# hahnyuan/PTQ4ViT

Hardware: AMD Instinct MI355X
Metric: calibration throughput (wrapped modules calibrated per second), ViT-B/224 W8A8, 32 calibration images (higher is better)
Workload: dtype int8

## Files before the change

include/ptq4vit_hip_debug.h:

```cpp
#ifndef PTQ4VIT_HIP_DEBUG_H
#define PTQ4VIT_HIP_DEBUG_H

#include <stdint.h>

#ifdef __cplusplus
extern "C" {
#endif

int p4v_debug_set_variant(int variant, int force_generic);
int p4v_debug_set_tuning(int key, int value);
int p4v_debug_topk_rows(const float* d_mass, int segs, int n, int k, int32_t* d_idx, void* stream);
int p4v_debug_pack_dual(const float* d_x, long rows, long cols, long cols_padded, int sos, int lo, int hi, int qmax,
                        const float* d_scale, float const_scale, int8_t* d_q1, int8_t* d_q2, void* stream);
int p4v_debug_pack_cands(const float* d_x, long rows, long cols, long rows_padded, long cols_padded, int layout, int lo, int hi,
                         const float* d_scales, int n_cands, const int* d_crange, const unsigned char* d_done, int live_max,
                         int general, int8_t* d_q, void* stream);
int p4v_debug_gather_im2col(int batch, int in_channels, int height, int width, int kernel_h, int kernel_w, int stride_h, int stride_w,
                            int pad_h, int pad_w, int dil_h, int dil_w, const float* d_x, const int32_t* d_idx, int k, float* d_dst,
                            void* stream);
int p4v_debug_prep_epi6(const float* d_o, const float* d_wt, const float* d_bias, long o_ss, long o_ts, int sr, int tr,
                        int bias_on_t, int wt_mode, int transposed, float* d_e, void* stream);

#ifdef __cplusplus
}
#endif
#endif
```

ptq4vit_amd/_lib.py:

```python
import ctypes as C
import os

_HERE = os.path.dirname(os.path.abspath(__file__))
LIB_PATH = os.environ.get("P4V_LIB") or os.path.join(_HERE, "csrc", "libptq4vit_hip.so")

METRICS = {
    "L1_norm": 0,
    "L2_norm": 1,
    "linear_weighted_L2_norm": 2,
    "square_weighted_L2_norm": 3,
    "hessian": 4,
    "cosine": 5,
}


class LinearDesc(C.Structure):
    _fields_ = [(n, C.c_int32) for n in (
        "batch", "tokens", "in_features", "out_features", "n_V", "n_H", "n_a", "w_bit", "a_bit", "metric",
        "eq_n", "search_round", "twin_postgelu", "init_layerwise", "has_bias", "reserved")]


class MatMulDesc(C.Structure):
    _fields_ = ([(n, C.c_int32) for n in ("batch", "heads", "M", "K", "N")] + [("_pad0", C.c_int32)] +
                [("a_stride", C.c_int64 * 4), ("b_stride", C.c_int64 * 4)] +
# ... 43 lines not shown
                ("scale1_stride", C.c_int64 * 4), ("scale1_div", C.c_int32 * 4),
                ("scale2_stride", C.c_int64 * 4), ("scale2_div", C.c_int32 * 4),
                ("scale2_const", C.c_float),
                ("mode", C.c_int32), ("lo1", C.c_int32), ("hi1", C.c_int32), ("lo2", C.c_int32), ("hi2", C.c_int32),
                ("qmax", C.c_int32), ("reserved", C.c_int32)]


class GroupJob(C.Structure):
    _fields_ = [("kind", C.c_int32), ("status", C.c_int32), ("desc", C.c_void_p), ("inp", C.c_void_p * 5), ("mult", C.c_void_p),
                ("out", C.c_void_p * 3), ("workspace", C.c_void_p), ("workspace_bytes", C.c_size_t)]


JOB_LINEAR, JOB_MATMUL, JOB_CONV, JOB_MATMUL_BLOCKS = 0, 1, 2, 3
PLANE_SYM, PLANE_SOS_HI, PLANE_SOS_LO, PLANE_TWIN = 1, 2, 3, 4
EXPORT_SYM_I8, EXPORT_SYM_F32, EXPORT_GELU_U8, EXPORT_SOS_U8 = 0, 1, 2, 3


EXPORTS = [
    "p4v_version", "p4v_last_error",
    "p4v_linear_workspace_bytes", "p4v_linear_calibrate",
    "p4v_matmul_workspace_bytes", "p4v_matmul_calibrate",
    "p4v_matmul_blocks_workspace_bytes", "p4v_matmul_blocks_calibrate", "p4v_amax_init_matmul_blocks",
    "p4v_matmul_blocks_search", "p4v_matmul_blocks_quant_forward",
    "p4v_conv_workspace_bytes", "p4v_conv_calibrate",
    "p4v_calibrate_group", "p4v_launch_counters",
    "p4v_linear_quant_forward", "p4v_matmul_quant_forward",
    "p4v_amax_init_linear", "p4v_linear_search_w", "p4v_linear_search_a",
    "p4v_amax_init_matmul", "p4v_matmul_search_A", "p4v_sos_search_split", "p4v_matmul_search_B",
    "p4v_amax_init_conv", "p4v_conv_search_w_channelwise", "p4v_conv_search_w_layerwise", "p4v_conv_search_a",
    "p4v_score_argmax_gather",
    "p4v_quantize_i8", "p4v_pack_plane_i8", "p4v_fake_quant", "p4v_export_quantize", "p4v_multi_copy",
    "p4v_stats_enable", "p4v_stats_reset", "p4v_stats_get", "p4v_stats_launches", "p4v_prune_counters",
    "p4v_debug_set_variant", "p4v_debug_set_tuning", "p4v_debug_topk_rows", "p4v_debug_pack_dual", "p4v_debug_prep_epi6",
    "p4v_debug_pack_cands", "p4v_debug_gather_im2col",
]

_lib = None


def load():
    global _lib
    if _lib is not None:
        return _lib
    if not os.path.exists(LIB_PATH):
        raise RuntimeError(
            f"ptq4vit_amd: HIP extension {LIB_PATH} is missing -- build it with "
            "`python -c 'import __graft_entry__ as g; g.build()'` (hipcc --offload-arch=gfx950). "
            "There is no CPU fallback for the calibration path.")
    import torch
    lib = C.CDLL(LIB_PATH)
    vp, fp, ip = C.c_void_p, C.c_void_p, C.c_void_p
    lib.p4v_version.restype = C.c_int
    lib.p4v_last_error.restype = C.c_char_p
    lib.p4v_linear_workspace_bytes.restype = C.c_size_t
    lib.p4v_linear_workspace_bytes.argtypes = [C.POINTER(LinearDesc)]
    lib.p4v_linear_calibrate.restype = C.c_int
    lib.p4v_linear_calibrate.argtypes = [C.POINTER(LinearDesc), fp, fp, fp, fp, fp, fp, fp, fp, fp, ip, vp, C.c_size_t, vp]
    lib.p4v_matmul_workspace_bytes.restype = C.c_size_t
    lib.p4v_matmul_workspace_bytes.argtypes = [C.POINTER(MatMulDesc)]
    lib.p4v_matmul_calibrate.restype = C.c_int
    lib.p4v_matmul_calibrate.argtypes = [C.POINTER(MatMulDesc), fp, fp, fp, fp, fp, fp, fp, fp, fp, ip, vp, C.c_size_t, vp]
    MBD = C.POINTER(MatMulBlocksDesc)
    lib.p4v_matmul_blocks_workspace_bytes.restype = C.c_size_t
    lib.p4v_matmul_blocks_workspace_bytes.argtypes = [MBD]
    lib.p4v_matmul_blocks_calibrate.restype = C.c_int
    lib.p4v_matmul_blocks_calibrate.argtypes = [MBD, fp, fp, fp, fp, fp, fp, fp, fp, fp, ip, vp, C.c_size_t, vp]
    lib.p4v_amax_init_matmul_blocks.restype = C.c_int
# ... 18 lines not shown
            ("p4v_linear_search_a", [LD] + [fp] * 9 + [ip]),
            ("p4v_amax_init_matmul", [MD] + [fp] * 4),
            ("p4v_matmul_search_A", [MD] + [fp] * 8 + [ip]),
            ("p4v_sos_search_split", [MD] + [fp] * 7 + [ip]),
            ("p4v_matmul_search_B", [MD] + [fp] * 9 + [ip]),
            ("p4v_amax_init_conv", [CD] + [fp] * 4),
            ("p4v_conv_search_w_channelwise", [CD] + [fp] * 9 + [ip]),
            ("p4v_conv_search_w_layerwise", [CD] + [fp] * 9 + [ip]),
            ("p4v_conv_search_a", [CD] + [fp] * 9 + [ip])):
        fn = getattr(lib, name)
        fn.restype = C.c_int
        fn.argtypes = args + tail
    lib.p4v_score_argmax_gather.restype = C.c_int
    lib.p4v_score_argmax_gather.argtypes = [fp, C.c_int32, C.c_int32, fp, fp, ip, vp]
    lib.p4v_quantize_i8.restype = C.c_int
    lib.p4v_quantize_i8.argtypes = [fp, C.c_int64, C.c_int64, C.c_int64, fp, C.c_int64, C.c_int32, C.c_int32, vp, vp]
    lib.p4v_fake_quant.restype = C.c_int
    lib.p4v_fake_quant.argtypes = [fp, C.c_int64, C.c_int64, fp, C.c_int64, C.c_int32, C.c_int32, fp, vp]
    lib.p4v_pack_plane_i8.restype = C.c_int
    lib.p4v_pack_plane_i8.argtypes = [C.POINTER(PlaneDesc), fp, fp, vp, vp]
    lib.p4v_export_quantize.restype = C.c_int
    lib.p4v_export_quantize.argtypes = [C.POINTER(ExportDesc), fp, fp, fp, vp, vp]
    lib.p4v_multi_copy.restype = C.c_int
    lib.p4v_multi_copy.argtypes = [vp, C.c_int32, C.c_int64, C.c_int64, vp]
    lib.p4v_debug_topk_rows.restype = C.c_int
    lib.p4v_debug_topk_rows.argtypes = [vp, C.c_int, C.c_int, C.c_int, vp, vp]
    lib.p4v_debug_pack_dual.restype = C.c_int
    lib.p4v_debug_pack_dual.argtypes = [fp, C.c_long, C.c_long, C.c_long, C.c_int, C.c_int, C.c_int, C.c_int, fp, C.c_float, vp, vp, vp]
    lib.p4v_debug_pack_cands.restype = C.c_int
    lib.p4v_debug_pack_cands.argtypes = [fp, C.c_long, C.c_long, C.c_long, C.c_long, C.c_int, C.c_int, C.c_int, fp, C.c_int, vp, vp,
                                         C.c_int, C.c_int, vp, vp]
    lib.p4v_debug_gather_im2col.restype = C.c_int
    lib.p4v_debug_gather_im2col.argtypes = [C.c_int] * 12 + [fp, ip, C.c_int, fp, vp]
    lib.p4v_debug_prep_epi6.restype = C.c_int
    lib.p4v_debug_prep_epi6.argtypes = [fp, fp, fp, C.c_long, C.c_long, C.c_int, C.c_int, C.c_int, C.c_int, C.c_int, fp, vp]
    lib.p4v_debug_set_variant.restype = C.c_int
    lib.p4v_debug_set_variant.argtypes = [C.c_int, C.c_int]
    lib.p4v_debug_set_tuning.restype = C.c_int
    lib.p4v_debug_set_tuning.argtypes = [C.c_int, C.c_int]
    lib.p4v_stats_enable.restype = C.c_int
    lib.p4v_stats_enable.argtypes = [C.c_int]
    lib.p4v_stats_reset.restype = C.c_int
    lib.p4v_stats_get.restype = C.c_int
    lib.p4v_stats_get.argtypes = [C.POINTER(KernelStats)]
    lib.p4v_stats_launches.restype = C.c_int
    lib.p4v_stats_launches.argtypes = [C.POINTER(LaunchRecord), C.c_int64, C.POINTER(C.c_int64)]
    lib.p4v_prune_counters.restype = C.c_int
    lib.p4v_prune_counters.argtypes = [C.POINTER(C.c_int64), C.c_int]
    lib.p4v_launch_counters.restype = C.c_int
    lib.p4v_launch_counters.argtypes = [C.POINTER(C.c_int64), C.c_int]
    lib.p4v_calibrate_group.restype = C.c_int
    lib.p4v_calibrate_group.argtypes = [C.POINTER(GroupJob), C.c_int32, vp, vp]
    _lib = lib
    return lib


def check(rc, what):
    if rc != 0:
        msg = load().p4v_last_error().decode("utf-8", "replace")
        if rc == -2:
            raise NotImplementedError(f"{what}: {msg}")
        raise RuntimeError(f"{what} failed (code {rc}): {msg}")


def source_hash():
    import hashlib
# ... 7 lines not shown
```

ptq4vit_amd/csrc/p4v_api.hip:

```cpp
#include <hip/hip_runtime.h>

#include <algorithm>
#include <atomic>
#include <climits>
#include <cstdarg>
#include <cstdio>
#include <condition_variable>
#include <cstring>
#include <deque>
#include <functional>
#include <thread>
#include <mutex>
#include <string>
#include <unordered_map>
#include <type_traits>
#include <vector>

#include "../../include/ptq4vit_hip.h"
#include "../../include/ptq4vit_hip_debug.h"
#include "p4v_kernels.h"

using namespace p4v;

namespace {
// ... 396 lines not shown
    for (auto& m : g_mir) if (m.dev == dev) return &m;
    return nullptr;
}
void attach_mirror(SelectParams& sl) {
    sl.iv_host = nullptr; sl.aux_host = nullptr;
    IvMirror* mi = mirror_of(sl.interval);
    IvMirror* ma = mirror_of(sl.aux_out);
    if (mi) mi->valid = false;
    if (ma) ma->valid = false;
    if (mi && sl.nj <= MIR_SLOT && sl.out_off == 0 && (sl.nj == 1 || sl.out_js == 1)) { sl.iv_host = mi->host; mi->valid = true; mi->count = sl.nj; }
    if (ma && sl.nj <= MIR_SLOT) { sl.aux_host = ma->host; ma->valid = true; ma->count = sl.nj; }
}

void metric_epi(int metric, int* epi, int* wt_mode) {
    switch (metric) {
        case P4V_METRIC_L1_NORM: *epi = EPI_ABS; *wt_mode = 0; break;
        case P4V_METRIC_L2_NORM: *epi = EPI_SQ; *wt_mode = 0; break;
        case P4V_METRIC_LINEAR_WEIGHTED_L2: *epi = EPI_W_SQ; *wt_mode = 3; break;
        case P4V_METRIC_SQUARE_WEIGHTED_L2: *epi = EPI_SQ_W; *wt_mode = 2; break;
        case P4V_METRIC_HESSIAN: *epi = EPI_SQ_W; *wt_mode = 1; break;
        default: *epi = EPI_COS; *wt_mode = 0; break;
    }
}

int launch_absmax(Ctx& c, const float* src, const long (&st)[4], int D0, int D1, int R, int C, int nV, int nH,
                  int crb_r, int crb_c, int signed_max, unsigned* out) {
    if (c.dry) return 0;
    CHK(q_fill(c, out, 0, sizeof(unsigned) * (size_t)D1 * nV * nH));
    AbsMaxParams p{src, st[0], st[1], st[2], st[3], D0, D1, R, C, nV, nH, crb_r, crb_c, 0, signed_max, out};
    p.row_tile = std::max(1, std::min(crb_r, std::max(1, 8192 / std::max(1, std::min(crb_c, C)))));
    const int tiles_per_v = cdiv(crb_r, p.row_tile);
    dim3 grid(tiles_per_v * nV * nH, D1, D0);
    return enqueue(c, KERN(AbsMaxParams, k_absmax), grid, dim3(256), 0, p);
}

int launch_interval(Ctx& c, const unsigned* enc, int n, float denom, int broadcast, float* interval) {
    if (c.dry) return 0;
    return enqueue(c, KERN(IntervalParams, k_interval_from_max), dim3(cdiv(n, 64)), dim3(64), 0, IntervalParams{enc, n, denom, broadcast, interval});
}

int launch_cands(Ctx& c, const float* mult, const float* interval, int ncand, int nblk, float* cands) {
    if (c.dry) return 0;
    return enqueue(c, KERN(CandsParams, k_make_cands), dim3(cdiv((long)ncand * nblk, 256)), dim3(256), 0, CandsParams{mult, interval, ncand, nblk, cands});
}

int launch_scale(Ctx& c, ScaleParams p) {
    if (c.dry) return 0;
    return enqueue(c, KERN(ScaleParams, k_scale_table), dim3(cdiv((long)p.C * p.nblk, 256)), dim3(256), 0, p);
}

std::atomic<int> g_cvt_state{0};
void cvt_probe(hipStream_t stream) {
    if (g_cvt_state.load(std::memory_order_acquire) != 0) return;
    static std::mutex mu;
    std::lock_guard<std::mutex> lk(mu);
    if (g_cvt_state.load(std::memory_order_acquire) != 0) return;
    static unsigned* scratch = nullptr;
    if (!scratch && hipMalloc(&scratch, 8 * sizeof(unsigned)) != hipSuccess) { (void)hipGetLastError(); scratch = nullptr; return; }
    unsigned h[5] = {9, 9, 9, 9, 9};
    hipLaunchKernelGGL(k_probe_cvt, dim3(1), dim3(64), 0, stream, scratch);
    if (hipGetLastError() != hipSuccess || hipMemcpyAsync(h, scratch, sizeof h, hipMemcpyDeviceToHost, stream) != hipSuccess ||
        hipStreamSynchronize(stream) != hipSuccess) { (void)hipGetLastError(); return; }
    const bool sat = h[3] == 0 && h[4] == 255;
    const int st = (sat && h[0] == 0 && h[1] == 1 && h[2] == 2) ? 1 : (sat && h[0] == 1 && h[1] == 2 && (h[2] == 2 || h[2] == 3)) ? 2 : 3;
    if (tune(TUNE_PRINT) > 0) fprintf(stderr, "[p4v] v_cvt_pk_u8_f32(0.7, 1.5, 2.5, -3, 300) = %u %u %u %u %u -> mode %d\n", h[0], h[1], h[2], h[3], h[4], st);
    g_cvt_state.store(st, std::memory_order_release);
// ... 862 lines not shown
    bool conv; PackParams conv_pk;
    int k_cap;
};
int slice_alloc(Ctx& c, SliceCache* sc, const SliceGeo& g, bool keep, bool bump) {
    if (sc->assigned) {
        if (sc->k != g.k_cap) return fail(P4V_ERR_INVALID, "slice cache reused with another geometry");
        return 0;
    }
    if (!keep && !bump) return 0;
    const long zrows = (long)g.segs * g.seg_rows, out_elems = (long)g.segs * g.k_cap * g.Ncols, row_elems = (long)g.segs * g.k_cap * g.K;
    if (keep) {
        sc->idx = reinterpret_cast<int*>(c.ws.get_top((size_t)g.segs * g.k_cap * sizeof(int)));
        sc->mass = reinterpret_cast<float*>(c.ws.get_top((size_t)zrows * sizeof(float)));
        sc->Os = reinterpret_cast<float*>(c.ws.get_top((size_t)out_elems * sizeof(float)));
        sc->Gs = reinterpret_cast<float*>(c.ws.get_top((size_t)out_elems * sizeof(float)));
        sc->Rs = reinterpret_cast<float*>(c.ws.get_top((size_t)row_elems * sizeof(float)));
        sc->frac = reinterpret_cast<float*>(c.ws.get_top(256));
        sc->assigned = true;
    } else {
        sc->idx = c.ws.get<int>((size_t)g.segs * g.k_cap);
        sc->mass = c.ws.get<float>((size_t)zrows);
        sc->Os = c.ws.get<float>((size_t)out_elems);
        sc->Gs = c.ws.get<float>((size_t)out_elems);
        sc->Rs = c.ws.get<float>((size_t)row_elems);
    }
    sc->k = g.k_cap;
    return 0;
}
int slice_fill(Ctx& c, SliceCache* sc, const SliceGeo& g, bool host_sync_ok) {
    const long zrows = (long)g.segs * g.seg_rows;
    const void* wsrc = g.G ? (const void*)g.G : (const void*)g.O;
    const bool new_idx = sc->idx_src != wsrc || sc->idx_wt != g.wt_mode || (g.wt_mode != 1 && sc->o_src != g.O);
    if (new_idx) {
        CHK(enqueue(c, KERN(RowMassParams, k_row_mass), dim3((unsigned)cdiv(zrows, 4)), dim3(256), 0, RowMassParams{g.G ? g.G : g.O, g.O, zrows, (long)g.Ncols, g.wt_mode, sc->mass}));
        CHK(enqueue(c, KERN(TopkParams, k_topk_rows), dim3(g.segs), dim3(1024), 0, TopkParams{sc->mass, g.seg_rows, g.k, sc->idx}));
        sc->idx_src = wsrc; sc->idx_wt = g.wt_mode;
        sc->o_src = sc->g_src = sc->r_src = nullptr;
        if (sc->frac && host_sync_ok && !(g_variant & 8388608)) {
            float f = 1.0f;
            int* hm = host_mirror(c);
            CHK(enqueue(c, KERN(MassFracParams, k_mass_fraction), dim3(1), dim3(1024), 0,
                        MassFracParams{sc->mass, zrows, sc->idx, g.segs, g.seg_rows, g.k, sc->frac, hm ? reinterpret_cast<float*>(hm + 4) : nullptr}));
            if (!hm) CHK(q_d2h(c, &f, sc->frac, sizeof f));
            CHK(q_sync(c));
            if (hm) f = *reinterpret_cast<volatile float*>(hm + 4);
            if (tune(TUNE_PRINT) > 0) fprintf(stderr, "[p4v] slice holds %.4f of the metric weight (%d x %d of %d rows)\n", f, g.segs, g.k, g.seg_rows);
            sc->frac_host = f;
            if (g.k < g.k_cap && !(f >= 0.97f)) {
                SliceGeo g2 = g;
                g2.k = g.k_cap;
                sc->idx_src = nullptr;
                return slice_fill(c, sc, g2, host_sync_ok);
            }
            const bool big_pass = zrows >= (tune(TUNE_LOOSE_ROWS) > 0 ? (long)tune(TUNE_LOOSE_ROWS) : 65536L);
            if (!(f >= (tune(TUNE_LOOSE_PCT) > 0 ? 0.01f * tune(TUNE_LOOSE_PCT) : big_pass ? 0.05f : 0.5f))) { sc->loose = true; return 0; }
        }
        sc->k_eff = g.k;
    }
    const int rows = g.segs * g.k;
    int gather_rc = 0;
    auto gather = [&](const float* src, long s0, long s3, int d3, float* dst, int seg, int zdiv, long sz2, long sz) {
        GatherParams gp{src, s0, 0, 0, s3, 1, 1, d3, sc->idx, rows, dst, seg, zdiv, sz2, sz};
        const long total = (long)rows * d3;
        if (const int r_ = enqueue(c, KERN(GatherParams, k_gather), dim3((unsigned)std::min<long>(cdiv(total, 256), 256L * 16)), dim3(256), 0, gp)) gather_rc = r_;
    };
    const int seg = g.lin ? 0 : g.k;
    const long o_seg = (long)g.seg_rows * g.Ncols;
    if (sc->o_src != g.O) { gather(g.O, g.o_ms, 1, g.Ncols, sc->Os, seg, 1, o_seg, 0); sc->o_src = g.O; }
    if (g.G && sc->g_src != g.G) { gather(g.G, g.o_ms, 1, g.Ncols, sc->Gs, seg, 1, o_seg, 0); sc->g_src = g.G; }
    if (sc->r_src != g.row_src) {
        if (g.conv) {
            const long total = (long)rows * g.K;
            CHK(enqueue(c, KERN(GatherIm2colParams, k_gather_im2col), dim3((unsigned)std::min<long>(cdiv(total, 256), 256L * 16)), dim3(256), 0, GatherIm2colParams{g.conv_pk, sc->idx, rows, sc->Rs}));
        } else if (g.lin) gather(g.row_src, g.s_r, 1, g.K, sc->Rs, 0, 1, 0, 0);
        else gather(g.row_src, g.s_r, g.s_k, g.K, sc->Rs, g.k, g.zdiv, g.s_z2, g.s_z);
        sc->r_src = g.row_src;
        sc->aplane.valid = false;
    }
    return gather_rc;
}

bool prune_ok(const Pass& ps) {
    if (!ps.prunable || !(ps.i8 || ps.prunable_f32) || ps.epi == EPI_COS || ps.store_out || ps.scores_out || ps.best_out || ps.crange || ps.no_select) return false;
    if ((g_variant & 4194304) || ps.eq_n < 32 || ps.nj < 1 || ps.nj > 4096) return false;
    return true;
}
int launch_pass_select(Ctx& c, const Pass& ps, const float* scores) {
    SelectParams sl{scores, ps.eq_n, ps.nj, ps.cands, ps.cand_cs, ps.cand_js, ps.cand_off, ps.interval, ps.out_js,
                    ps.out_off, ps.aux_out, ps.aux_div, ps.scores_out, ps.scores_out_ld, ps.best_out};
    return launch_select(c, sl);
}

#define PRUNE_COUNT(i) do { if (!c.dry) g_prune_cnt[i].fetch_add(1, std::memory_order_relaxed); } while (0)
constexpr int PRUNE_FP32_CHAIN = 128 + 6;
inline float prune_margin() { return std::max(1e-4f, 4.0f * 2.0f * (float)PRUNE_FP32_CHAIN * 5.9604645e-8f); }
int prune_crosscheck_begin(Ctx& c, const float* interval, int n, std::vector<float>& keep) {
    keep.resize(n);
// ... 1833 lines not shown
    Ctx c{(hipStream_t)stream, Arena(nullptr, 0), false};
    cvt_bias(c);
    PackParams p = pack2d(d_x, rows, cols, cols);
    p.Rp = (int)rows_padded; p.Kp = (int)cols_padded; p.dst = d_q; p.C = n_cands; p.c_inner = layout;
    p.scales = d_scales; p.sc_cs = 1; p.lo = lo; p.hi = hi;
    p.crange = d_crange; p.c_base = 0; p.done = d_done;
    g_pack_general.store(general ? 1 : 0, std::memory_order_relaxed);
    const int r = launch_pack<int8_t>(c, p, live_max);
    g_pack_general.store(0, std::memory_order_relaxed);
    return r;
}

int p4v_debug_gather_im2col(int batch, int in_channels, int height, int width, int kernel_h, int kernel_w, int stride_h, int stride_w,
                            int pad_h, int pad_w, int dil_h, int dil_w, const float* d_x, const int32_t* d_idx, int k, float* d_dst,
                            void* stream) {
    if (!d_x || !d_idx || !d_dst || k <= 0 || batch <= 0 || in_channels <= 0 || height <= 0 || width <= 0 || kernel_h <= 0 ||
        kernel_w <= 0 || stride_h <= 0 || stride_w <= 0 || pad_h < 0 || pad_w < 0 || dil_h <= 0 || dil_w <= 0)
        return fail(P4V_ERR_INVALID, "p4v_debug_gather_im2col: bad argument");
    const int num_h = height + 2 * pad_h - dil_h * (kernel_h - 1) - 1, num_w = width + 2 * pad_w - dil_w * (kernel_w - 1) - 1;
    if (num_h < 0 || num_w < 0) return fail(P4V_ERR_INVALID, "p4v_debug_gather_im2col: bad geometry");
    const int fh = num_h / stride_h + 1, fw = num_w / stride_w + 1;
    PackParams p{};
    p.src = d_x; p.conv = 1; p.ic = in_channels; p.H = height; p.W = width; p.kh = kernel_h; p.kw = kernel_w;
    p.sh = stride_h; p.sw = stride_w; p.ph = pad_h; p.pw = pad_w; p.dh = dil_h; p.dw = dil_w;
    p.fw = fw; p.L = fh * fw;
    p.Z = 1; p.s_z = 0; p.R = batch * fh * fw; p.K = in_channels * kernel_h * kernel_w; p.nblk_r = 1; p.nblk_k = 1;
    p.mode = PACK_RAW;
    Ctx c{(hipStream_t)stream, Arena(nullptr, 0), false};
    const long total = (long)k * p.K;
    return enqueue(c, KERN(GatherIm2colParams, k_gather_im2col), dim3((unsigned)std::min<long>(cdiv(total, 256), 256L * 16)), dim3(256), 0,
                   GatherIm2colParams{p, d_idx, k, d_dst});
}

int p4v_debug_prep_epi6(const float* d_o, const float* d_wt, const float* d_bias, long o_ss, long o_ts, int sr, int tr,
                        int bias_on_t, int wt_mode, int transposed, float* d_e, void* stream) {
    if (!d_o || !d_bias || !d_e || (wt_mode == 1 && !d_wt) || sr <= 0 || tr <= 0 || wt_mode < 0 || wt_mode > 4)
        return fail(P4V_ERR_INVALID, "p4v_debug_prep_epi6: bad argument");
    PrepEpi6Params pe{};
    pe.O = d_o; pe.Wt = d_wt ? d_wt : d_o; pe.bias = d_bias; pe.o_ss = o_ss; pe.o_ts = o_ts; pe.SR = sr; pe.TR = tr;
    pe.bias_on_t = bias_on_t ? 1 : 0; pe.wt_mode = wt_mode; pe.transposed = transposed ? 1 : 0;
    pe.stiles = cdiv(sr, 256); pe.ttiles = cdiv(tr, 64); pe.E = d_e;
    Ctx c{(hipStream_t)stream, Arena(nullptr, 0), false};
    return enqueue(c, KERN(PrepEpi6Params, k_prep_epi6), dim3((unsigned)std::min<long>((long)pe.stiles * pe.ttiles, 256L * 32)), dim3(256), 0, pe);
}

int p4v_pack_plane_i8(const p4v_plane_desc* d, const float* d_x, const float* d_scales, int8_t* d_q, void* stream) {
    if (!d || !d_x || !d_q || d->rows <= 0 || d->cols <= 0 || d->cols_padded % 64 || d->cols_padded < d->cols)
        return fail(P4V_ERR_INVALID, "p4v_pack_plane_i8: bad argument");
    if (d->mode != P4V_PLANE_SYM && d->mode != P4V_PLANE_SOS_HI && d->mode != P4V_PLANE_SOS_LO && d->mode != P4V_PLANE_TWIN)
        return fail(P4V_ERR_INVALID, "p4v_pack_plane_i8: unknown mode %d", d->mode);
    if (d->mode == P4V_PLANE_TWIN && (d->lo > 0 || d->hi < 0 || !(d->const_scale > 0.0f)))
        return fail(P4V_ERR_INVALID, "p4v_pack_plane_i8: the merged twin plane needs lo <= 0 <= hi and const_scale > 0");
    if (d->mode != P4V_PLANE_SYM && !d_scales) return fail(P4V_ERR_INVALID, "p4v_pack_plane_i8: split-of-softmax planes need d_scales = &split");
    if (d->mode == P4V_PLANE_SYM && d_scales && d->rows_per_scale <= 0) return fail(P4V_ERR_INVALID, "p4v_pack_plane_i8: rows_per_scale");
    if (d->lo < -128 || d->hi > 127 || d->qmax < 2 || d->qmax > 128) return fail(P4V_ERR_INVALID, "p4v_pack_plane_i8: grid wider than int8");
    Ctx c{(hipStream_t)stream, Arena(nullptr, 0), false};
    cvt_bias(c);
    PackParams p = pack2d(d_x, d->rows, d->cols, d->cols);
    p.Rp = (int)d->rows; p.Kp = (int)d->cols_padded; p.dst = d_q; p.C = 1;
    p.scales = d_scales; p.sc_cs = 0; p.neg_scale = d->const_scale;
    p.lo = d->lo; p.hi = d->hi; p.qm1 = (float)(d->qmax - 1);
    if (d->mode == P4V_PLANE_SYM) {
        p.mode = PACK_SYM;
        if (d_scales) { p.blk_mode = 1; p.blk_div = (int)d->rows_per_scale; p.nblk_r = cdiv(d->rows, d->rows_per_scale); p.nblk_k = 1; }
    } else if (d->mode == P4V_PLANE_TWIN) {
        p.mode = PACK_TWIN_I8;
// ... 34 lines not shown
```

ptq4vit_amd/csrc/p4v_kernels.h:

```cpp
#pragma once
#include <hip/hip_runtime.h>
#include <stdint.h>
#include <type_traits>

namespace p4v {

typedef int v4i __attribute__((ext_vector_type(4)));
typedef int v16i __attribute__((ext_vector_type(16)));
typedef float v4f __attribute__((ext_vector_type(4)));
typedef float v16f __attribute__((ext_vector_type(16)));
typedef float v2f __attribute__((ext_vector_type(2)));

#ifndef P4V_GROUP_KERNARG
#define P4V_GROUP_KERNARG (4096 - 256)
#endif
template <typename P> struct GroupArgs {
    static constexpr int CAP_RAW = (P4V_GROUP_KERNARG - 16) / (int)(sizeof(P) + 16);
    static constexpr int CAP = CAP_RAW > 64 ? 64 : CAP_RAW;
    int n;
    unsigned off[CAP + 1];
    unsigned gx[CAP], gy[CAP], gz[CAP];
    P p[CAP];
};
#define P4V_BIDX uint3{blockIdx.x, blockIdx.y, blockIdx.z}
// ... 18 lines not shown

struct AbsMaxParams {
    const float* src;
    long s0, s1, s2, s3;
    int D0, D1, R, C;
    int nV, nH, crb_r, crb_c;
    int row_tile;
    int signed_max;
    unsigned* out;
};

__device__ __forceinline__ void k_absmax_body(const AbsMaxParams& p, const uint3 blockIdx, const uint3 gridDim) {
    int bx = blockIdx.x;
    const int h = bx % p.nH; bx /= p.nH;
    const int v = bx % p.nV; bx /= p.nV;
    const int rt = bx;
    const int r0 = v * p.crb_r + rt * p.row_tile;
    const int r1 = min(min(r0 + p.row_tile, (v + 1) * p.crb_r), p.R);
    const int c0 = h * p.crb_c;
    const int c1 = min(c0 + p.crb_c, p.C);
    const int w = c1 - c0;
    const float* base = p.src + (long)blockIdx.z * p.s0 + (long)blockIdx.y * p.s1;
    float m = -INFINITY;
    if (w > 0 && r1 > r0 && p.s3 == 1 && (w & 3) == 0 && (p.s2 & 3) == 0 && (c0 & 3) == 0 && ((((unsigned long long)base) & 15) == 0)) {
        const int w4 = w >> 2;
        const int tpr = w4 >= 256 ? 256 : w4 >= 128 ? 128 : w4 >= 64 ? 64 : w4 >= 32 ? 32 : 16;
        const int tx = threadIdx.x & (tpr - 1), ty = threadIdx.x / tpr, rpar = 256 / tpr;
        for (int r = r0 + ty; r < r1; r += rpar) {
            const v4f* row = reinterpret_cast<const v4f*>(base + (long)r * p.s2 + c0);
            for (int c = tx; c < w4; c += tpr) {
                const v4f x = row[c];
                if (p.signed_max) m = fmaxf(fmaxf(m, fmaxf(x[0], x[1])), fmaxf(x[2], x[3]));
                else m = fmaxf(fmaxf(m, fmaxf(fabsf(x[0]), fabsf(x[1]))), fmaxf(fabsf(x[2]), fabsf(x[3])));
            }
        }
    } else if (w > 0 && r1 > r0) {
        const int n = (r1 - r0) * w;
        for (int i = threadIdx.x; i < n; i += 256) {
            const int r = r0 + i / w, c = c0 + i % w;
            float x = base[(long)r * p.s2 + (long)c * p.s3];
            m = fmaxf(m, p.signed_max ? x : fabsf(x));
        }
    }
    for (int o = 32; o > 0; o >>= 1) m = fmaxf(m, __shfl_xor(m, o));
    __shared__ float red[4];
    if ((threadIdx.x & 63) == 0) red[threadIdx.x >> 6] = m;
    __syncthreads();
    if (threadIdx.x == 0) {
        m = fmaxf(fmaxf(red[0], red[1]), fmaxf(red[2], red[3]));
        if (m > -INFINITY) atomicMax(p.out + ((long)blockIdx.y * p.nV + v) * p.nH + h, enc_ordered(m));
    }
}
__global__ __launch_bounds__(256) void k_absmax(AbsMaxParams p) { k_absmax_body(p, P4V_BIDX, P4V_GDIM); }
__global__ __launch_bounds__(256) void k_absmax_g(GroupArgs<AbsMaxParams> a) { P4V_GROUP_ENTER(a); k_absmax_body(a.p[m_], vb_, vg_); }

struct IntervalParams { const unsigned* enc; int n; float denom; int broadcast; float* interval; };
__device__ __forceinline__ void k_interval_from_max_body(const IntervalParams& a, const uint3 blockIdx, const uint3 gridDim) {
    const auto& [enc, n, denom, broadcast, interval] = a;
    int j = blockIdx.x * blockDim.x + threadIdx.x;
    if (j >= n) return;
    float m;
    if (broadcast) {
        m = -INFINITY;
        for (int i = 0; i < n; ++i) m = fmaxf(m, dec_ordered(enc[i]));
    } else {
        m = dec_ordered(enc[j]);
// ... 3430 lines not shown
    if (p.j_mode == 3) {
        const int smp = j * nt + threadIdx.x;
        if (smp < p.S) {
            for (int zb = 0; zb < p.ZB; ++zb) acc += (double)cos_item(p, c, zb, 0, p.ZV, smp);
            p.scores[(long)c * p.nj + smp] = (float)(p.norm * acc);
        }
        return;
    }
    int zv0 = 0, zv1 = p.ZV, zlo = 0, zstep = 1;
    if (p.j_mode == 1) { zv0 = j; zv1 = j + 1; }
    if (p.j_mode == 2) { zlo = j; zstep = p.j_div; }
    const int nz = (p.ZB - zlo + zstep - 1) / zstep;
    const long total = (long)nz * p.S;
    for (long i = threadIdx.x; i < total; i += nt) {
        const int smp = (int)(i % p.S);
        const int zb = zlo + (int)(i / p.S) * zstep;
        acc += (double)cos_item(p, c, zb, zv0, zv1, smp);
    }
    __shared__ double red[1024];
    red[threadIdx.x] = acc;
    __syncthreads();
    for (int o = nt >> 1; o > 0; o >>= 1) {
        if (threadIdx.x < o) red[threadIdx.x] += red[threadIdx.x + o];
        __syncthreads();
    }
    if (threadIdx.x == 0) p.scores[(long)c * p.nj + j] = (float)(p.norm * red[0]);
}
__global__ __launch_bounds__(1024) void k_finish_cos(FinishCosParams p) { k_finish_cos_body(p, P4V_BIDX, P4V_GDIM); }
__global__ __launch_bounds__(1024) void k_finish_cos_g(GroupArgs<FinishCosParams> a) { P4V_GROUP_ENTER(a); k_finish_cos_body(a.p[m_], vb_, vg_); }

struct RowMassParams { const float* W; const float* O; long rows; long cols; int wt_mode; float* mass; };
__device__ __forceinline__ void k_row_mass_body(const RowMassParams& a_, const uint3 blockIdx, const uint3 gridDim) {
    const auto& [W, O, rows, cols, wt_mode, mass] = a_;
    const long r = (long)blockIdx.x * 4 + (threadIdx.x >> 6);
    if (r >= rows) return;
    const int lane = threadIdx.x & 63;
    const float* src = (wt_mode == 1 ? W : O) + r * cols;
    float s = 0.0f;
    if (wt_mode == 0) s = lane == 0 ? 1.0f : 0.0f;
    else
        for (long i = lane; i < cols; i += 64) {
            const float v = src[i];
            s += wt_mode == 2 ? fabsf(v) : v * v;
        }
    for (int o = 32; o > 0; o >>= 1) s += __shfl_xor(s, o);
    if (lane == 0) mass[r] = s;
}
__global__ __launch_bounds__(256) void k_row_mass(RowMassParams p) { k_row_mass_body(p, P4V_BIDX, P4V_GDIM); }
__global__ __launch_bounds__(256) void k_row_mass_g(GroupArgs<RowMassParams> a) { P4V_GROUP_ENTER(a); k_row_mass_body(a.p[m_], vb_, vg_); }
__global__ void k_group_mass(const float* mass, int n_groups, int group, float* out) {
    const int g = blockIdx.x * blockDim.x + threadIdx.x;
    if (g >= n_groups) return;
    float s = 0.0f;
    for (int i = 0; i < group; ++i) s += mass[(long)g * group + i];
    out[g] = s;
}
struct TopkParams { const float* mass_all; int n; int k; int* idx_all; };
__device__ __forceinline__ void k_topk_rows_body(const TopkParams& a_, const uint3 blockIdx, const uint3 gridDim) {
    const auto& [mass_all, n, k, idx_all] = a_;
    const float* mass = mass_all + (long)blockIdx.x * n;
    int* idx = idx_all + (long)blockIdx.x * k;
    __shared__ int hist[256];
    __shared__ int wtot[4];
    __shared__ int wg[2][16], we[2][16];
    __shared__ unsigned prefix_s;
    __shared__ int krem_s;
    const int t = threadIdx.x, lane = t & 63, wv = t >> 6;
    auto key = [&](int i) -> unsigned { const unsigned b = __float_as_uint(mass[i]); return (b & 0x80000000u) ? 0u : b; };
    if (t == 0) { prefix_s = 0; krem_s = k; }
    for (int shift = 24; shift >= 0; shift -= 8) {
        if (t < 256) hist[t] = 0;
        __syncthreads();
        const unsigned hi_mask = shift == 24 ? 0u : (0xFFFFFFFFu << (shift + 8));
        const unsigned pre = prefix_s;
        const int kr = krem_s;
        for (int i0 = 0; i0 < n; i0 += 1024) {
            const int i = i0 + t;
            const unsigned kv = i < n ? key(i) : 0u;
            const bool in = i < n && (kv & hi_mask) == pre;
// ... 41 lines not shown
        const bool take = is_gt || (is_eq && eq_before < eq_room);
        if (take) idx[base + gt_before + min(eq_before, eq_room)] = i;
        const int eq_take = min(eq_tot, eq_room);
        base += gt_tot + eq_take;
        eq_taken += eq_take;
    }
}
__global__ __launch_bounds__(1024) void k_topk_rows(TopkParams p) { k_topk_rows_body(p, P4V_BIDX, P4V_GDIM); }
__global__ __launch_bounds__(1024) void k_topk_rows_g(GroupArgs<TopkParams> a) { P4V_GROUP_ENTER(a); k_topk_rows_body(a.p[m_], vb_, vg_); }
struct MassFracParams { const float* mass; long n; const int* idx; int segs; int seg_rows; int k; float* frac; float* frac_host; };
__device__ __forceinline__ void k_mass_fraction_body(const MassFracParams& a_, const uint3 blockIdx, const uint3 gridDim) {
    const auto& [mass, n, idx, segs, seg_rows, k, frac, frac_host] = a_;
    __shared__ double red[1024];
    double tot = 0.0, sel = 0.0;
    for (long i = threadIdx.x; i < n; i += 1024) tot += (double)mass[i];
    for (long i = threadIdx.x; i < (long)segs * k; i += 1024) sel += (double)mass[(i / k) * seg_rows + idx[i]];
    for (int pass = 0; pass < 2; ++pass) {
        red[threadIdx.x] = pass ? sel : tot;
        __syncthreads();
        for (int o = 512; o > 0; o >>= 1) { if (threadIdx.x < o) red[threadIdx.x] += red[threadIdx.x + o]; __syncthreads(); }
        if (threadIdx.x == 0) { if (pass) sel = red[0]; else tot = red[0]; }
        __syncthreads();
    }
    if (threadIdx.x == 0) {
        const float f = tot > 0.0 ? (float)(sel / tot) : 0.0f;
        frac[0] = f;
        if (frac_host) frac_host[0] = f;
    }
}
__global__ __launch_bounds__(1024) void k_mass_fraction(MassFracParams p) { k_mass_fraction_body(p, P4V_BIDX, P4V_GDIM); }
__global__ __launch_bounds__(1024) void k_mass_fraction_g(GroupArgs<MassFracParams> a) { P4V_GROUP_ENTER(a); k_mass_fraction_body(a.p[m_], vb_, vg_); }

struct GatherParams { const float* src; long s0, s1, s2, s3; int d1, d2, d3; const int* idx; int k; float* dst; int seg, zdiv; long sz2, sz; };
__device__ __forceinline__ void k_gather_body(const GatherParams& p, const uint3 blockIdx, const uint3 gridDim) {
    const long inner = (long)p.d1 * p.d2 * p.d3, total = inner * p.k;
    for (long i = (long)blockIdx.x * 256 + threadIdx.x; i < total; i += (long)gridDim.x * 256) {
        const int r = (int)(i / inner);
        long rem = i - (long)r * inner;
        const int a = (int)(rem / ((long)p.d2 * p.d3)); rem -= (long)a * p.d2 * p.d3;
        const int b = (int)(rem / p.d3), cidx = (int)(rem - (long)b * p.d3);
        long off = 0;
        if (p.seg > 0) { const int z = r / p.seg; off = (long)(z / p.zdiv) * p.sz2 + (long)(z % p.zdiv) * p.sz; }
        p.dst[i] = p.src[off + (long)p.idx[r] * p.s0 + (long)a * p.s1 + (long)b * p.s2 + (long)cidx * p.s3];
    }
}
__global__ __launch_bounds__(256) void k_gather(GatherParams p) { k_gather_body(p, P4V_BIDX, P4V_GDIM); }
__global__ __launch_bounds__(256) void k_gather_g(GroupArgs<GatherParams> a) { P4V_GROUP_ENTER(a); k_gather_body(a.p[m_], vb_, vg_); }

struct GatherIm2colParams { PackParams p; const int* idx; int k; float* dst; };
__device__ __forceinline__ void k_gather_im2col_body(const GatherIm2colParams& a_, const uint3 blockIdx, const uint3 gridDim) {
    const auto& [p, idx, k, dst] = a_;
    const long total = (long)k * p.K;
    for (long i = (long)blockIdx.x * 256 + threadIdx.x; i < total; i += (long)gridDim.x * 256) {
        const int r = (int)(i / p.K), kk = (int)(i - (long)r * p.K);
        dst[i] = pack_load(p, p.src, idx[r], kk);
    }
}
__global__ __launch_bounds__(256) void k_gather_im2col(GatherIm2colParams p) { k_gather_im2col_body(p, P4V_BIDX, P4V_GDIM); }
__global__ __launch_bounds__(256) void k_gather_im2col_g(GroupArgs<GatherIm2colParams> a) { P4V_GROUP_ENTER(a); k_gather_im2col_body(a.p[m_], vb_, vg_); }
struct NchwRowsParams { const float* src; int oc; int L; float* dst; };
__device__ __forceinline__ void k_nchw_to_rows_body(const NchwRowsParams& a_, const uint3 blockIdx, const uint3 gridDim) {
    const auto& [src, oc, L, dst] = a_;
    __shared__ float t[32][33];
    const int l0 = blockIdx.x * 32, c0 = blockIdx.y * 32, bi = blockIdx.z;
    const int tx = threadIdx.x & 31, ty = threadIdx.x >> 5;
    for (int i = ty; i < 32; i += 8)
        if (c0 + i < oc && l0 + tx < L) t[i][tx] = src[((long)bi * oc + c0 + i) * L + l0 + tx];
// ... 342 lines not shown
```

ptq4vit_amd/engine.py:

```python
import ctypes as C

import torch

from . import _lib

_workspace = {}
_mult_cache = {}


def _require_cuda(t, what):
    if not t.is_cuda:
        raise RuntimeError(f"ptq4vit_amd: {what} must live on the GPU (got {t.device}); the calibration path has no CPU fallback")


def device_of(*tensors):
    for t in tensors:
        if t is not None and t.is_cuda:
            return t.device
    if not torch.cuda.is_available():
        raise RuntimeError("ptq4vit_amd: no GPU visible -- the HIP calibration engine needs an MI355X (no CPU fallback)")
    return torch.device("cuda", torch.cuda.current_device())


def to_dev(t, dev):
# ... 635 lines not shown
    rows, cols = x2d.shape
    n = scales.numel()
    colsp = (cols + 63) // 64 * 64
    rowsp = rows if rows_padded is None else int(rows_padded)
    size = rowsp * colsp * (1 if layout == 3 else (n + 1) // 2 * 2 if layout == 2 else n)
    if out is None:
        out = torch.zeros(size, dtype=torch.int8, device=x2d.device)
    assert out.dtype == torch.int8 and out.is_contiguous() and out.numel() >= size
    with torch.cuda.device(x2d.device):
        rc = _lib.load().p4v_debug_pack_cands(ptr(x2d), rows, cols, rowsp, colsp, int(layout), int(lo), int(hi), ptr(scales), n,
                                              ptr(crange) if crange is not None else None,
                                              ptr(done) if done is not None else None, int(live_max), int(bool(general)),
                                              ptr(out), stream_ptr(x2d.device))
    _lib.check(rc, "p4v_debug_pack_cands")
    return out


def debug_gather_im2col(x, idx, *, kernel_size, stride, padding, dilation):
    assert x.is_cuda and x.dtype == torch.float32 and x.dim() == 4 and idx.is_cuda and idx.dtype == torch.int32 and idx.dim() == 1
    x, idx = x.contiguous(), idx.contiguous()
    b, ic, H, W = x.shape
    (kh, kw), (sh, sw), (ph, pw), (dh, dw) = kernel_size, stride, padding, dilation
    fh, fw = (H + 2 * ph - dh * (kh - 1) - 1) // sh + 1, (W + 2 * pw - dw * (kw - 1) - 1) // sw + 1
    if fh > 0 and fw > 0:
        assert idx.numel() > 0 and int(idx.min()) >= 0 and int(idx.max()) < b * fh * fw, "row index outside the im2col matrix"
    out = torch.full((idx.numel(), ic * kh * kw), float("nan"), dtype=torch.float32, device=x.device)
    with torch.cuda.device(x.device):
        rc = _lib.load().p4v_debug_gather_im2col(b, ic, H, W, kh, kw, sh, sw, ph, pw, dh, dw, ptr(x), ptr(idx), idx.numel(), ptr(out),
                                                 stream_ptr(x.device))
    _lib.check(rc, "p4v_debug_gather_im2col")
    return out


def debug_prep_epi6(o, wt, bias, *, o_ss, o_ts, sr, tr, bias_on_t, wt_mode, transposed):
    n = -(-sr // 256) * -(-tr // 64) * 256 * 64 * 2
    e = torch.full((n,), float("nan"), dtype=torch.float32, device=o.device)
    with torch.cuda.device(o.device):
        rc = _lib.load().p4v_debug_prep_epi6(ptr(o), ptr(wt) if wt is not None else None, ptr(bias), int(o_ss), int(o_ts),
                                             int(sr), int(tr), int(bias_on_t), int(wt_mode), int(transposed), ptr(e),
                                             stream_ptr(o.device))
    _lib.check(rc, "p4v_debug_prep_epi6")
    return e

def stats_reset():
    _lib.load().p4v_stats_reset()


def stats_get():
    s = _lib.KernelStats()
    _lib.check(_lib.load().p4v_stats_get(C.byref(s)), "p4v_stats_get")
    return {k: getattr(s, k) for k, _ in _lib.KernelStats._fields_}


def prune_counters(reset=False):
    out = (C.c_int64 * 4)()
    _lib.check(_lib.load().p4v_prune_counters(out, int(bool(reset))), "p4v_prune_counters")
    return dict(zip(("staged", "staged_no_survivors", "kept_full_sweep", "not_eligible"), (int(v) for v in out)))


def stats_launches():
    lib = _lib.load()
    n = C.c_int64(0)
    _lib.check(lib.p4v_stats_launches(None, 0, C.byref(n)), "p4v_stats_launches")
    buf = (_lib.LaunchRecord * max(1, n.value))()
    _lib.check(lib.p4v_stats_launches(buf, n.value, C.byref(n)), "p4v_stats_launches")
    return [{"kernel": _lib.LAUNCH_KINDS.get(r.kind, str(r.kind)), "stage": _lib.LAUNCH_STAGES.get(r.stage, str(r.stage)),
# ... 3 lines not shown
```

Measured before the change: 677.3.

## Vectorize row gather, batch row-mass loads, add strided absmax path

Rewrites k_row_mass as a grid-stride loop. For short rows it loads four rows per wave at once, and for long rows it unrolls the column loads eight deep. k_gather gets a row-wise path that handles four gathered rows per unit, using float4 loads when the strides and pointers are aligned. k_absmax gets a new branch for unit-stride columns that reads four rows per iteration with a thread width matched to the tile width. Debug entry points are added to test each kernel on its own. The aim is more memory-level parallelism and wider transactions in these bandwidth-bound helper kernels, at the cost of more branches and more register pressure.

```diff
diff --git a/include/ptq4vit_hip_debug.h b/include/ptq4vit_hip_debug.h
--- a/include/ptq4vit_hip_debug.h
+++ b/include/ptq4vit_hip_debug.h
@@ -20,6 +20,11 @@
                             void* stream);
 int p4v_debug_prep_epi6(const float* d_o, const float* d_wt, const float* d_bias, long o_ss, long o_ts, int sr, int tr,
                         int bias_on_t, int wt_mode, int transposed, float* d_e, void* stream);
+int p4v_debug_row_mass(const float* d_w, long rows, long cols, int wt_mode, float* d_mass, void* stream);
+int p4v_debug_gather(const float* d_src, long s0, long s3, int d3, const int32_t* d_idx, int k, int seg, int zdiv, long sz2, long sz,
+                     float* d_dst, void* stream);
+int p4v_debug_absmax(const float* d_src, const int64_t* strides4, int d0, int d1, int rows, int cols, int n_v, int n_h, int signed_max,
+                     uint32_t* d_enc, void* stream);
 
 #ifdef __cplusplus
 }
diff --git a/ptq4vit_amd/_lib.py b/ptq4vit_amd/_lib.py
--- a/ptq4vit_amd/_lib.py
+++ b/ptq4vit_amd/_lib.py
@@ -99,7 +99,7 @@
     "p4v_quantize_i8", "p4v_pack_plane_i8", "p4v_fake_quant", "p4v_export_quantize", "p4v_multi_copy",
     "p4v_stats_enable", "p4v_stats_reset", "p4v_stats_get", "p4v_stats_launches", "p4v_prune_counters",
     "p4v_debug_set_variant", "p4v_debug_set_tuning", "p4v_debug_topk_rows", "p4v_debug_pack_dual", "p4v_debug_prep_epi6",
-    "p4v_debug_pack_cands", "p4v_debug_gather_im2col",
+    "p4v_debug_pack_cands", "p4v_debug_gather_im2col", "p4v_debug_row_mass", "p4v_debug_gather", "p4v_debug_absmax",
 ]
 
 _lib = None
@@ -184,6 +184,12 @@
                                          C.c_int, C.c_int, vp, vp]
     lib.p4v_debug_gather_im2col.restype = C.c_int
     lib.p4v_debug_gather_im2col.argtypes = [C.c_int] * 12 + [fp, ip, C.c_int, fp, vp]
+    lib.p4v_debug_row_mass.restype = C.c_int
+    lib.p4v_debug_row_mass.argtypes = [fp, C.c_long, C.c_long, C.c_int, fp, vp]
+    lib.p4v_debug_gather.restype = C.c_int
+    lib.p4v_debug_gather.argtypes = [fp, C.c_long, C.c_long, C.c_int, ip, C.c_int, C.c_int, C.c_int, C.c_long, C.c_long, fp, vp]
+    lib.p4v_debug_absmax.restype = C.c_int
+    lib.p4v_debug_absmax.argtypes = [fp, C.POINTER(C.c_int64)] + [C.c_int] * 7 + [vp, vp]
     lib.p4v_debug_prep_epi6.restype = C.c_int
     lib.p4v_debug_prep_epi6.argtypes = [fp, fp, fp, C.c_long, C.c_long, C.c_int, C.c_int, C.c_int, C.c_int, C.c_int, fp, vp]
     lib.p4v_debug_set_variant.restype = C.c_int
diff --git a/ptq4vit_amd/csrc/p4v_api.hip b/ptq4vit_amd/csrc/p4v_api.hip
--- a/ptq4vit_amd/csrc/p4v_api.hip
+++ b/ptq4vit_amd/csrc/p4v_api.hip
@@ -452,6 +452,21 @@
     const int tiles_per_v = cdiv(crb_r, p.row_tile);
     dim3 grid(tiles_per_v * nV * nH, D1, D0);
     return enqueue(c, KERN(AbsMaxParams, k_absmax), grid, dim3(256), 0, p);
+}
+
+int launch_row_mass(Ctx& c, const float* W, const float* O, long rows, long cols, int wt_mode, float* mass) {
+    const long waves = wt_mode != 0 && cols <= 256 ? cdiv(rows, 4) : rows;
+    return enqueue(c, KERN(RowMassParams, k_row_mass), dim3((unsigned)std::min<long>(cdiv(waves, 4), 2048L)), dim3(256), 0,
+                   RowMassParams{W, O, rows, cols, wt_mode, mass});
+}
+int launch_gather(Ctx& c, const GatherParams& gp) {
+    long blocks = cdiv((long)gp.k * gp.d1 * gp.d2 * gp.d3, 256);
+    if (gather_rows_ok(gp)) {
+        const GatherShape gs = gather_shape(gp);
+        if (gs.units >= (1L << 31)) return fail(P4V_ERR_UNSUPPORTED, "slice too large for k_gather (%ld row units)", gs.units);
+        blocks = cdiv(gs.units, gs.per_wg);
+    }
+    return enqueue(c, KERN(GatherParams, k_gather), dim3((unsigned)std::min<long>(blocks, 256L * 16)), dim3(256), 0, gp);
 }
 
 int launch_interval(Ctx& c, const unsigned* enc, int n, float denom, int broadcast, float* interval) {
@@ -1380,7 +1395,7 @@
     const void* wsrc = g.G ? (const void*)g.G : (const void*)g.O;
     const bool new_idx = sc->idx_src != wsrc || sc->idx_wt != g.wt_mode || (g.wt_mode != 1 && sc->o_src != g.O);
     if (new_idx) {
-        CHK(enqueue(c, KERN(RowMassParams, k_row_mass), dim3((unsigned)cdiv(zrows, 4)), dim3(256), 0, RowMassParams{g.G ? g.G : g.O, g.O, zrows, (long)g.Ncols, g.wt_mode, sc->mass}));
+        CHK(launch_row_mass(c, g.G ? g.G : g.O, g.O, zrows, (long)g.Ncols, g.wt_mode, sc->mass));
         CHK(enqueue(c, KERN(TopkParams, k_topk_rows), dim3(g.segs), dim3(1024), 0, TopkParams{sc->mass, g.seg_rows, g.k, sc->idx}));
         sc->idx_src = wsrc; sc->idx_wt = g.wt_mode;
         sc->o_src = sc->g_src = sc->r_src = nullptr;
@@ -1409,8 +1424,7 @@
     int gather_rc = 0;
     auto gather = [&](const float* src, long s0, long s3, int d3, float* dst, int seg, int zdiv, long sz2, long sz) {
         GatherParams gp{src, s0, 0, 0, s3, 1, 1, d3, sc->idx, rows, dst, seg, zdiv, sz2, sz};
-        const long total = (long)rows * d3;
-        if (const int r_ = enqueue(c, KERN(GatherParams, k_gather), dim3((unsigned)std::min<long>(cdiv(total, 256), 256L * 16)), dim3(256), 0, gp)) gather_rc = r_;
+        if (const int r_ = launch_gather(c, gp)) gather_rc = r_;
     };
     const int seg = g.lin ? 0 : g.k;
     const long o_seg = (long)g.seg_rows * g.Ncols;
@@ -3310,6 +3324,28 @@
                    GatherIm2colParams{p, d_idx, k, d_dst});
 }
 
+int p4v_debug_row_mass(const float* d_w, long rows, long cols, int wt_mode, float* d_mass, void* stream) {
+    if (!d_w || !d_mass || rows <= 0 || cols <= 0 || wt_mode < 0 || wt_mode > 3) return fail(P4V_ERR_INVALID, "p4v_debug_row_mass: bad argument");
+    Ctx c{(hipStream_t)stream, Arena(nullptr, 0), false};
+    return launch_row_mass(c, d_w, d_w, rows, cols, wt_mode, d_mass);
+}
+
+int p4v_debug_gather(const float* d_src, long s0, long s3, int d3, const int32_t* d_idx, int k, int seg, int zdiv, long sz2, long sz,
+                     float* d_dst, void* stream) {
+    if (!d_src || !d_idx || !d_dst || d3 <= 0 || k <= 0 || seg < 0 || zdiv <= 0) return fail(P4V_ERR_INVALID, "p4v_debug_gather: bad argument");
+    Ctx c{(hipStream_t)stream, Arena(nullptr, 0), false};
+    return launch_gather(c, GatherParams{d_src, s0, 0, 0, s3, 1, 1, d3, d_idx, k, d_dst, seg, zdiv, sz2, sz});
+}
+
+int p4v_debug_absmax(const float* d_src, const int64_t* strides4, int d0, int d1, int rows, int cols, int n_v, int n_h, int signed_max,
+                     uint32_t* d_enc, void* stream) {
+    if (!d_src || !strides4 || !d_enc || d0 <= 0 || d1 <= 0 || rows <= 0 || cols <= 0 || n_v <= 0 || n_h <= 0)
+        return fail(P4V_ERR_INVALID, "p4v_debug_absmax: bad argument");
+    Ctx c{(hipStream_t)stream, Arena(nullptr, 0), false};
+    const long st[4] = {(long)strides4[0], (long)strides4[1], (long)strides4[2], (long)strides4[3]};
+    return launch_absmax(c, d_src, st, d0, d1, rows, cols, n_v, n_h, cdiv(rows, n_v), cdiv(cols, n_h), signed_max ? 1 : 0, d_enc);
+}
+
 int p4v_debug_prep_epi6(const float* d_o, const float* d_wt, const float* d_bias, long o_ss, long o_ts, int sr, int tr,
                         int bias_on_t, int wt_mode, int transposed, float* d_e, void* stream) {
     if (!d_o || !d_bias || !d_e || (wt_mode == 1 && !d_wt) || sr <= 0 || tr <= 0 || wt_mode < 0 || wt_mode > 4)
diff --git a/ptq4vit_amd/csrc/p4v_kernels.h b/ptq4vit_amd/csrc/p4v_kernels.h
--- a/ptq4vit_amd/csrc/p4v_kernels.h
+++ b/ptq4vit_amd/csrc/p4v_kernels.h
@@ -74,6 +74,20 @@
                 const v4f x = row[c];
                 if (p.signed_max) m = fmaxf(fmaxf(m, fmaxf(x[0], x[1])), fmaxf(x[2], x[3]));
                 else m = fmaxf(fmaxf(m, fmaxf(fabsf(x[0]), fabsf(x[1]))), fmaxf(fabsf(x[2]), fabsf(x[3])));
+            }
+        }
+    } else if (w > 0 && r1 > r0 && p.s3 == 1) {
+        const int tpr = w >= 256 ? 256 : w >= 128 ? 128 : w >= 64 ? 64 : w >= 32 ? 32 : 16;
+        const int tx = threadIdx.x & (tpr - 1), ty = threadIdx.x / tpr, rpar = 256 / tpr;
+        const float* col = base + c0;
+        for (int r = r0 + ty; r < r1; r += 4 * rpar) {
+            const float* row = col + (long)r * p.s2;
+            const long rs = (long)rpar * p.s2;
+            const bool h1 = r + rpar < r1, h2 = r + 2 * rpar < r1, h3 = r + 3 * rpar < r1;
+            for (int c = tx; c < w; c += tpr) {
+                float x0 = row[c], x1 = h1 ? row[rs + c] : x0, x2 = h2 ? row[2 * rs + c] : x0, x3 = h3 ? row[3 * rs + c] : x0;
+                if (!p.signed_max) { x0 = fabsf(x0); x1 = fabsf(x1); x2 = fabsf(x2); x3 = fabsf(x3); }
+                m = fmaxf(fmaxf(m, fmaxf(x0, x1)), fmaxf(x2, x3));
             }
         }
     } else if (w > 0 && r1 > r0) {
@@ -3570,19 +3584,49 @@
 struct RowMassParams { const float* W; const float* O; long rows; long cols; int wt_mode; float* mass; };
 __device__ __forceinline__ void k_row_mass_body(const RowMassParams& a_, const uint3 blockIdx, const uint3 gridDim) {
     const auto& [W, O, rows, cols, wt_mode, mass] = a_;
-    const long r = (long)blockIdx.x * 4 + (threadIdx.x >> 6);
-    if (r >= rows) return;
     const int lane = threadIdx.x & 63;
-    const float* src = (wt_mode == 1 ? W : O) + r * cols;
-    float s = 0.0f;
-    if (wt_mode == 0) s = lane == 0 ? 1.0f : 0.0f;
-    else
-        for (long i = lane; i < cols; i += 64) {
-            const float v = src[i];
-            s += wt_mode == 2 ? fabsf(v) : v * v;
-        }
-    for (int o = 32; o > 0; o >>= 1) s += __shfl_xor(s, o);
-    if (lane == 0) mass[r] = s;
+    const long wave = (long)blockIdx.x * 4 + (threadIdx.x >> 6), waves = (long)gridDim.x * 4;
+    const float* src = wt_mode == 1 ? W : O;
+    const bool absw = wt_mode == 2;
+    auto finish = [&](float s, long r) {
+        for (int o = 32; o > 0; o >>= 1) s += __shfl_xor(s, o);
+        if (lane == 0) mass[r] = s;
+    };
+    if (wt_mode == 0) {
+        for (long r = wave; r < rows; r += waves) finish(lane == 0 ? 1.0f : 0.0f, r);
+    } else if (cols <= 256) {
+        const int nc = (int)cols;
+        for (long q = wave; q * 4 < rows; q += waves) {
+            float v[4][4];
+#pragma unroll
+            for (int j = 0; j < 4; ++j) {
+                const long r = q * 4 + j;
+                const float* row = src + r * cols;
+#pragma unroll
+                for (int t = 0; t < 4; ++t) { const int i = lane + 64 * t; v[j][t] = (r < rows && i < nc) ? row[i] : 0.0f; }
+            }
+#pragma unroll
+            for (int j = 0; j < 4; ++j) {
+                float s = 0.0f;
+#pragma unroll
+                for (int t = 0; t < 4; ++t) s += absw ? fabsf(v[j][t]) : v[j][t] * v[j][t];
+                if (q * 4 + j < rows) finish(s, q * 4 + j);
+            }
+        }
+    } else {
+        for (long r = wave; r < rows; r += waves) {
+            const float* row = src + r * cols;
+            float s = 0.0f;
+            for (long i0 = lane; i0 < cols; i0 += 512) {
+                float v[8];
+#pragma unroll
+                for (int t = 0; t < 8; ++t) { const long i = i0 + 64 * t; v[t] = i < cols ? row[i] : 0.0f; }
+#pragma unroll
+                for (int t = 0; t < 8; ++t) s += absw ? fabsf(v[t]) : v[t] * v[t];
+            }
+            finish(s, r);
+        }
+    }
 }
 __global__ __launch_bounds__(256) void k_row_mass(RowMassParams p) { k_row_mass_body(p, P4V_BIDX, P4V_GDIM); }
 __global__ __launch_bounds__(256) void k_row_mass_g(GroupArgs<RowMassParams> a) { P4V_GROUP_ENTER(a); k_row_mass_body(a.p[m_], vb_, vg_); }
@@ -3690,7 +3734,61 @@
 __global__ __launch_bounds__(1024) void k_mass_fraction_g(GroupArgs<MassFracParams> a) { P4V_GROUP_ENTER(a); k_mass_fraction_body(a.p[m_], vb_, vg_); }
 
 struct GatherParams { const float* src; long s0, s1, s2, s3; int d1, d2, d3; const int* idx; int k; float* dst; int seg, zdiv; long sz2, sz; };
+__host__ __device__ inline bool gather_rows_ok(const GatherParams& p) { return p.s3 == 1 && p.d1 == 1 && p.d2 == 1; }
+__host__ __device__ inline bool gather_vec_ok(const GatherParams& p) {
+    return ((p.d3 | p.s0 | (p.seg > 0 ? (p.sz2 | p.sz) : 0L)) & 3) == 0 && (((unsigned long long)p.src | (unsigned long long)p.dst) & 15) == 0;
+}
+struct GatherShape { int n, G, chunks; long units; int per_wg; };
+__host__ __device__ inline GatherShape gather_shape(const GatherParams& p) {
+    GatherShape g;
+    const bool vec = gather_vec_ok(p);
+    g.n = vec ? p.d3 / 4 : p.d3;
+    g.G = g.n <= 32 ? 32 : 64;
+    const int chunk = g.G * (vec ? 2 : 4);
+    g.chunks = (g.n + chunk - 1) / chunk;
+    g.units = (long)((p.k + 3) / 4) * g.chunks;
+    g.per_wg = 256 / g.G;
+    return g;
+}
+template <typename V, int STEPS>
+__device__ __forceinline__ void gather_rows(const GatherParams& p, const GatherShape& g, const uint3 blockIdx, const uint3 gridDim) {
+    const int sl = threadIdx.x & (g.G - 1);
+    const V* src = reinterpret_cast<const V*>(p.src);
+    V* dst = reinterpret_cast<V*>(p.dst);
+    constexpr int VW = sizeof(V) / 4;
+    for (long u = (long)blockIdx.x * g.per_wg + threadIdx.x / g.G; u < g.units; u += (long)gridDim.x * g.per_wg) {
+        const int q = (int)((unsigned)u / (unsigned)g.chunks), c0 = (int)(u - (long)q * g.chunks) * g.G * STEPS + sl;
+        long so[4];
+        bool ok[4];
+#pragma unroll
+        for (int j = 0; j < 4; ++j) {
+            const int r = q * 4 + j;
+            ok[j] = r < p.k;
+            long off = 0;
+            if (ok[j]) {
+                if (p.seg > 0) { const int z = r / p.seg; off = (long)(z / p.zdiv) * p.sz2 + (long)(z % p.zdiv) * p.sz; }
+                off += (long)p.idx[r] * p.s0;
+            }
+            so[j] = off / VW;
+        }
+        V v[4][STEPS];
+#pragma unroll
+        for (int j = 0; j < 4; ++j)
+#pragma unroll
+            for (int t = 0; t < STEPS; ++t) { const int c = c0 + t * g.G; if (ok[j] && c < g.n) v[j][t] = src[so[j] + c]; }
+#pragma unroll
+        for (int j = 0; j < 4; ++j)
+#pragma unroll
+            for (int t = 0; t < STEPS; ++t) { const int c = c0 + t * g.G; if (ok[j] && c < g.n) dst[(long)(q * 4 + j) * g.n + c] = v[j][t]; }
+    }
+}
 __device__ __forceinline__ void k_gather_body(const GatherParams& p, const uint3 blockIdx, const uint3 gridDim) {
+    if (gather_rows_ok(p)) {
+        const GatherShape g = gather_shape(p);
+        if (gather_vec_ok(p)) gather_rows<v4f, 2>(p, g, blockIdx, gridDim);
+        else gather_rows<float, 4>(p, g, blockIdx, gridDim);
+        return;
+    }
     const long inner = (long)p.d1 * p.d2 * p.d3, total = inner * p.k;
     for (long i = (long)blockIdx.x * 256 + threadIdx.x; i < total; i += (long)gridDim.x * 256) {
         const int r = (int)(i / inner);
diff --git a/ptq4vit_amd/engine.py b/ptq4vit_amd/engine.py
--- a/ptq4vit_amd/engine.py
+++ b/ptq4vit_amd/engine.py
@@ -691,6 +691,37 @@
     return out
 
 
+def debug_row_mass(w, rows, cols, wt_mode, mass):
+    assert w.is_cuda and w.dtype == torch.float32 and w.is_contiguous() and w.numel() >= rows * cols
+    assert mass.is_cuda and mass.dtype == torch.float32 and mass.is_contiguous() and mass.numel() >= rows
+    with torch.cuda.device(w.device):
+        rc = _lib.load().p4v_debug_row_mass(ptr(w), int(rows), int(cols), int(wt_mode), ptr(mass), stream_ptr(w.device))
+    _lib.check(rc, "p4v_debug_row_mass")
+    return mass
+
+
+def debug_gather(src, idx, dst, *, s0, s3, d3, seg=0, zdiv=1, sz2=0, sz=0):
+    assert src.is_cuda and src.dtype == torch.float32 and src.is_contiguous() and dst.dtype == torch.float32 and dst.is_contiguous()
+    assert idx.is_cuda and idx.dtype == torch.int32 and idx.dim() == 1 and idx.is_contiguous() and dst.numel() >= idx.numel() * d3
+    with torch.cuda.device(src.device):
+        rc = _lib.load().p4v_debug_gather(ptr(src), int(s0), int(s3), int(d3), ptr(idx), idx.numel(), int(seg), int(zdiv), int(sz2),
+                                          int(sz), ptr(dst), stream_ptr(src.device))
+    _lib.check(rc, "p4v_debug_gather")
+    return dst
+
+
+def debug_absmax(x, *, n_v=1, n_h=1, signed_max=False):
+    assert x.is_cuda and x.dtype == torch.float32 and x.dim() == 4
+    d0, d1, rows, cols = x.shape
+    st = (C.c_int64 * 4)(*x.stride())
+    enc = torch.full((d1, n_v, n_h), 0x7FFFFFFF, dtype=torch.int32, device=x.device)
+    with torch.cuda.device(x.device):
+        rc = _lib.load().p4v_debug_absmax(ptr(x), st, d0, d1, rows, cols, int(n_v), int(n_h), int(bool(signed_max)), ptr(enc),
+                                          stream_ptr(x.device))
+    _lib.check(rc, "p4v_debug_absmax")
+    return enc
+
+
 def debug_prep_epi6(o, wt, bias, *, o_ss, o_ts, sr, tr, bias_on_t, wt_mode, transposed):
     n = -(-sr // 256) * -(-tr // 64) * 256 * 64 * 2
     e = torch.full((n,), float("nan"), dtype=torch.float32, device=o.device)
```

Result: slower. 669.8 (-1.1%).
